# OmerMersin/video-stab

Measured on AMD Instinct MI355X. Metric: stabilized frames/sec @1080p (whole job; warp-stage HBM GB/s in roofline), higher is better.
Workload: dtype u8

## Files before the change

### video-stab_amd/csrc/batch_schedule.cpp

```cpp
#include <cstring>
#include <new>

#include "stab_internal.h"

using namespace vsd;

struct vs_batch {
    int device = 0, S = 0, B = 0, cap = 0;
    bool own = false;
    std::vector<vs_stab*> m;
    vs_stab* ref = nullptr;
    std::string err;
    FirstFailure failure;
    hipStream_t st = nullptr, st_pre = nullptr, st_det = nullptr, st_up = nullptr;
    bool allocated = false;
    uint8_t* h_tables = nullptr;
    size_t h_set_bytes = 0, ho_pairs = 0, ho_lk = 0, ho_rs = 0, ho_tail = 0, ho_gf = 0, ho_seg = 0;
    uint8_t* d_all = nullptr;
    uint8_t *d_lk[2] = {nullptr, nullptr}, *d_rs[2] = {nullptr, nullptr}, *d_tail[2] = {nullptr, nullptr}, *d_seg[2] = {nullptr, nullptr}, *d_gf = nullptr;
    uint8_t* d_tin[2] = {nullptr, nullptr};
    ImgPair* d_pairs[2] = {nullptr, nullptr};
    size_t up_bytes = 0;
    int pre_rel_step = -1;
    double* d_MinvB[2] = {nullptr, nullptr};
// ... 190 lines not shown
};

int fill_stream_items(vs_batch* g, vs_stab* s, const vs_batch::HostSet& H, const BorderPlan& bp, int ndue, int first, StepPlan& P) {
    const vs_params_c& p = s->p;
    const int ns = (int)s->bq.size(), dset = g->dev_set(P.k), set = g->pend_set;
    vs_batch::Ready& R = g->next;
    int npad = 0;
    for (int i = 0; i < ns; i++) {
        const int idx = first + i;
        const vs_stab::BFrame& b = s->bq[i];
        const vs_stab::ItemBufs& it = s->items[i];
        LKLevel L[MAX_PYR];
        fill_lk_levels(s, b.pv, b.c, L);
        const int cap = std::max(b.lk_cap, 0);
        P.n_max = std::max(P.n_max, cap);
        uint8_t *rs = H.rs + ransac_item_bytes() * idx, *tail = H.tail + tail_item_bytes() * idx;
        VS_OBJ_TRY(g, lk_fill_item(H.lk + lk_item_bytes() * idx, L, s->levels, s->d_pts[b.lk_buf], cap, s->d_npts[b.lk_buf], it.next, it.status, it.err,
                              p.lk_win_size, p.lk_max_iters, p.lk_epsilon));
        VS_OBJ_TRY(g, ransac_fill_item(rs, s->d_pts[b.lk_buf], it.next, it.status, cap, s->d_npts[b.lk_buf], it.vp, it.vc, it.m, 4, p.ransac_threshold,
                                  p.ransac_max_iters, s->tab, it.counts, it.model, it.inliers, it.info, s->d_traj, &s->tp, s->d_dbg, b.have_prev_gray));
        ransac_item_set_last(rs, i == ns - 1 ? 1 : 0);
        ransac_item_set_tail_in(rs, g->d_tin[dset] + tail_in_bytes() * idx);
        double* minv = nullptr;
        WarpTabJob jobs[2] = {{nullptr, nullptr, nullptr, 0, 0}, {nullptr, nullptr, nullptr, 0, 0}};
        if (b.out_due) {
            const int j = P.npend++;
            minv = g->d_MinvB[set] + 12 * j;
            R.srcs[j] = b.out_frame; R.dsts[j] = b.d_out; R.slots[j] = b.out_slot; R.owner[j] = s; R.pad_idx[j] = npad;
            if (P.all_apart && std::min(WARP_BATCH_MAX, ndue - j / WARP_BATCH_MAX * WARP_BATCH_MAX) >= WARP_TAB_MIN) {
                const WarpEnds e = warp_ends(s, b.out_frame, b.d_out, npad, bp);
                int32_t* T = g->d_tabs[set] + (size_t)j * g->tab_ints;
                jobs[0] = WarpTabJob{T, e.src, e.dst, bp.pw, bp.ph};
                if (fmt_two_planes(s->fmt))
                    jobs[1] = WarpTabJob{T + tab_layout(s->w, s->h).stride, e.src + src_uv(s), e.dst + dst_uv(s, e.dst, b.out_stride), s->w / 2, s->h / 2};
                else if (fmt_three_planes(s->fmt))
                    jobs[1] = WarpTabJob{T + tab_layout(s->w, s->h).stride, e.src + src_i420(s).u, e.dst + dst_i420(s, e.dst, b.out_stride).u, s->w / 2, s->h / 2};
            }
            npad++;
            P.pend_stride = b.out_stride;
        }
        tail_fill_item(tail, b.out_due ? 1 : 0, b.out_idx, minv, jobs);
        tail_item_set_seg(tail, P.nseg);
    }
    tail_fill_seg(H.seg + tail_seg_bytes() * P.nseg, first, ns, s->d_M, s->d_traj, s->d_dbg, p.smoothing_method);
    P.any_apart |= p.smoothing_method != VS_SMOOTH_KALMAN;
    P.nseg++;
    return VS_OK;
}

void fill_pair_tables(const vs_batch* g, const std::vector<vs_stab*>& act, ImgPair* h_pairs, StepPlan& P) {
    const int L = g->ref->levels;
    int n_first = 0, n_rest = 0, i = 0;
    for (vs_stab* s : act)
        for (const vs_stab::BFrame& b : s->bq) {
            const Pyramid& py = s->pyr[b.c];
            const int slot = b.detect ? n_first++ : P.ndet + n_rest++;
            h_pairs[slot] = ImgPair{b.frame, py.img[0]};
            if ((uintptr_t)b.frame % 8) P.aligned = 0;
            for (int l = 1; l <= L; l++) h_pairs[(size_t)l * P.n + i] = ImgPair{py.img[l - 1], py.img[l]};
// ... 356 lines not shown
```

### video-stab_amd/csrc/k_ransac.hip

```cpp
#include <map>
#include <mutex>
#include <vector>

#include <cstring>

#include "traj_device.h"
#include "traj_emit_device.h"
#include "vs_common.h"
#include "warp_tab.h"

namespace vsd {

struct RansacTables {
    int max_m = 0, iters = 0;
    uint32_t* d_pairs = nullptr;
    uint32_t* d_update = nullptr;
};

namespace {

struct CvRng {
    uint64_t state;
    explicit CvRng(uint64_t s) : state(s ? s : 0xffffffffULL) {}
    uint32_t next() {
// ... 508 lines not shown
                     iters, tab, d_counts, d_model, d_inliers, d_info, traj, tp, dbg, have_prev_gray);
    return VS_OK;
}

int launch_ransac_score_batch(const void* d_table, int items, int iters, int n_max, hipStream_t st) {
    if (!d_table || items < 1 || items > 65535 || iters < 1 || n_max < 0 || n_max > MAX_PTS) {
        set_last_error("ransac_score_batch: invalid argument");
        return VS_ERR_INVALID_ARG;
    }
    hipLaunchKernelGGL(ransac_score16_batch_kernel, dim3((iters + SC_HYP - 1) / SC_HYP, items), dim3(64), (size_t)(n_max > 0 ? n_max : 1) * 16, st,
                       static_cast<const RansacArgs*>(d_table));
    hipLaunchKernelGGL(ransac_select_batch_kernel, dim3(items), dim3(64), 0, st, static_cast<const RansacArgs*>(d_table), items - 1);
    VS_HIP_TRY(hipGetLastError());
    return VS_OK;
}

size_t tail_item_bytes() { return sizeof(TailItem); }

void tail_fill_item(void* host_item, int out_due, int out_idx, double* d_Minv_out, const WarpTabJob* tabs) {
    TailItem& t = *static_cast<TailItem*>(host_item);
    t.out_due = out_due; t.out_idx = out_idx; t.Minv_out = d_Minv_out; t.ncnt = 0; t.seg = 0;
    for (int i = 0; i < 2; i++) {
        if (tabs) t.tab[i] = tabs[i];
        else { t.tab[i].tabs = nullptr; t.tab[i].src = nullptr; t.tab[i].dst = nullptr; t.tab[i].dw = 0; t.tab[i].dh = 0; }
    }
}

size_t tail_seg_bytes() { return sizeof(TailSeg); }
void tail_fill_seg(void* host_seg, int first, int n, float* d_M_out, TrajState* traj, vs_debug_frame* dbg, int smoothing_method) {
    TailSeg& g = *static_cast<TailSeg*>(host_seg);
    g.first = first; g.n = n; g.M_out = d_M_out; g.traj = traj; g.dbg = dbg;
    g.apart = smoothing_method != VS_SMOOTH_KALMAN ? 1 : 0; g.pad = 0;
}
size_t tail_in_bytes() { return sizeof(TailIn); }
void tail_in_fill(void* host_tail_in, const double* model, int ok, int nprev, int have_prev_gray) {
    TailIn& t = *static_cast<TailIn*>(host_tail_in);
    memset(&t, 0, sizeof t);
    for (int i = 0; i < 6; i++) t.model[i] = ok ? model[i] : __builtin_nan("");
    t.info[0] = ok; t.info[1] = ok ? 0 : -1;
    t.nprev = nprev; t.have_prev_gray = have_prev_gray;
}
void ransac_fill_item_traj(void* host_item, TrajState* traj, const TrajParams* tp, vs_debug_frame* dbg) {
    RansacArgs& a = *static_cast<RansacArgs*>(host_item);
    memset(&a, 0, sizeof a);
    a.traj = traj; a.tp = *tp; a.dbg = dbg; a.have_prev_gray = 1;
}
void ransac_item_set_tail_in(void* host_item, void* d_tail_in) { static_cast<RansacArgs*>(host_item)->tail_in = static_cast<TailIn*>(d_tail_in); }
// ... 58 lines not shown
```

### video-stab_amd/csrc/k_warp.hip

```cpp
#include <algorithm>
#include <cstdlib>
#include <map>
#include <mutex>
#include <utility>
#include <vector>

#include "launchers.h"
#include "vs_common.h"
#include "warp_tab.h"

namespace vsd {

namespace {

constexpr int TW = WT_TW;
constexpr int TH = WT_TH;
constexpr int PX = 4;
constexpr int NT = 256;
constexpr int TXN = TW / PX;
constexpr int TYN = NT / TXN;
constexpr int MAXB = WARP_BATCH_MAX;
constexpr int FDATA = 136;
constexpr int FPITCH = 136;
constexpr int FROWS = 25;
constexpr int LDS_PX = FPITCH * FROWS;
constexpr int SG = FDATA / 4;
constexpr int SR = 7;
constexpr int SPASS = (FROWS + SR - 1) / SR;
constexpr int LUT_STRIDE = 32;
constexpr int OBUF = (NT / 64) * 2 * TW;

struct WarpCore {
    size_t sstride, dstride;
    int sw, sh, dw, dh;
    int src_aligned, dst_aligned;
    int border;
};

struct WarpArgs {
    WarpCore c;
    const double* Minv_dev;
    double Minv_val[MAXB * 6];
    int minv_stride;
    int32_t* tabs;
    int tab_stride;
    int tab_row, tab_ad;
    const uint8_t* srcs[MAXB];
    uint8_t* dsts[MAXB];
};

template <int CN, int SB = 1>
__device__ __forceinline__ uint32_t load_px_checked(const uint8_t* src, size_t sstride, int sw,
                                                    int sh, int sx, int sy, int border = VS_BORDER_BLACK) {
    if (border == VS_BORDER_REPLICATE) {
        sx = sx < 0 ? 0 : (sx >= sw ? sw - 1 : sx);
        sy = sy < 0 ? 0 : (sy >= sh ? sh - 1 : sy);
    } else if ((unsigned)sx >= (unsigned)sw || (unsigned)sy >= (unsigned)sh) return 0u;
    if (SB == 2) {
        const uint16_t* q = reinterpret_cast<const uint16_t*>(src + (size_t)sy * sstride) + (size_t)sx * CN;
        uint32_t v16 = q[0];
        if (CN > 1) v16 |= (uint32_t)q[1] << 16;
        return v16;
    }
    const uint8_t* p = src + (size_t)sy * sstride + (size_t)sx * CN;
    uint32_t v = p[0];
    if (CN > 1) v |= (uint32_t)p[1] << 8;
    if (CN > 2) v |= (uint32_t)p[2] << 16;
    if (CN > 3) v |= (uint32_t)p[3] << 24;
    return v;
// ... 272 lines not shown
}

__device__ __forceinline__ int coord_term(double p, double q, double v) { return wt_coord_term(p, q, v); }

__device__ __forceinline__ void load_map(const WarpArgs& a, int bz, double* m) {
    if (a.Minv_dev) {
        const __attribute__((address_space(4))) double* mp =
            (const __attribute__((address_space(4))) double*)(a.Minv_dev + a.minv_stride * bz);
#pragma unroll
        for (int i = 0; i < 6; i++) m[i] = mp[i];
    } else {
#pragma unroll
        for (int i = 0; i < 6; i++) m[i] = a.Minv_val[6 * bz + i];
    }
}

constexpr int TAB_COL = WT_COL;

__global__ __launch_bounds__(NT) void warp_tables_kernel(WarpArgs a) {
    const int bz = blockIdx.y;
    double m[6];
    load_map(a, bz, m);
    TabLayout L;
    L.row = a.tab_row; L.ad = a.tab_ad; L.stride = a.tab_stride;
    const int j = blockIdx.x * NT + threadIdx.x;
    if (j < wt_entries(a.c.dw, a.c.dh))
        wt_build_entry(a.tabs + (size_t)bz * a.tab_stride, L, m, a.c.dw, a.c.dh, a.srcs[bz], a.dsts[bz], j);
}

constexpr int NVT_MAX = 16;
struct NvTabArgs {
    int32_t* tabs;
    int block, chroma;
    int w, h;
    size_t src_uv, dst_uv;
    const uint8_t* ys[NVT_MAX];
    uint8_t* yd[NVT_MAX];
    double my[NVT_MAX * 6], muv[NVT_MAX * 6];
};

__global__ __launch_bounds__(NT) void warp_tables_nv12_kernel(NvTabArgs a) {
    const int bz = blockIdx.y, plane = blockIdx.z;
    const int dw = plane ? a.w / 2 : a.w, dh = plane ? a.h / 2 : a.h;
    TabLayout L = tab_layout(dw, dh);
    L.stride = a.block;
    double m[6];
#pragma unroll
    for (int i = 0; i < 6; i++) m[i] = plane ? a.muv[6 * bz + i] : a.my[6 * bz + i];
    const int j = blockIdx.x * NT + threadIdx.x;
    if (j < wt_entries(dw, dh))
// ... 36 lines not shown
        } else if (tid < 2 * 64 + TH) {
            const int r = min(y0 + (tid - 128), y1);
            tv0 = Tg[2 * a.c.dw + r]; tv1 = Tg[2 * a.c.dw + a.c.dh + r];
        }
    } else {
        double m[6];
        load_map(a, bz, m);
        if (wave < 2) {
            const double dv = (double)min(x0 + tid, x1);
            s_ad[tid] = coord_term(m[0], 0.0, dv);
            s_bd[tid] = coord_term(m[3], 0.0, dv);
        } else if (tid < 2 * 64 + TH) {
            const double dv = (double)min(y0 + (tid - 128), y1);
            s_x0[tid - 128] = coord_term(m[1], m[2], dv) + 16;
            s_y0[tid - 128] = coord_term(m[4], m[5], dv) + 16;
        }
        __syncthreads();
        const int cl = x1 - x0, rl = y1 - y0;
        ad0 = __builtin_amdgcn_readfirstlane(s_ad[0]); ad1 = __builtin_amdgcn_readfirstlane(s_ad[cl]);
        bd0 = __builtin_amdgcn_readfirstlane(s_bd[0]); bd1 = __builtin_amdgcn_readfirstlane(s_bd[cl]);
        Xa = __builtin_amdgcn_readfirstlane(s_x0[0]); Xb = __builtin_amdgcn_readfirstlane(s_x0[rl]);
        Ya = __builtin_amdgcn_readfirstlane(s_y0[0]); Yb = __builtin_amdgcn_readfirstlane(s_y0[rl]);
    }
    int bx0, bx1, by0, by1;
    bool saturated;
    {
        const int sx00 = (Xa + ad0) >> 10, sx01 = (Xa + ad1) >> 10, sx10 = (Xb + ad0) >> 10, sx11 = (Xb + ad1) >> 10;
        const int sy00 = (Ya + bd0) >> 10, sy01 = (Ya + bd1) >> 10, sy10 = (Yb + bd0) >> 10, sy11 = (Yb + bd1) >> 10;
        const int rx0 = min(min(sx00, sx01), min(sx10, sx11)), rx1 = max(max(sx00, sx01), max(sx10, sx11));
        const int ry0 = min(min(sy00, sy01), min(sy10, sy11)), ry1 = max(max(sy00, sy01), max(sy10, sy11));
        saturated = rx0 < -32768 || ry0 < -32768 || rx1 > 32767 || ry1 > 32767;
        bx0 = max(rx0, -32768); bx1 = min(rx1, 32767) + 1;
        by0 = max(ry0, -32768); by1 = min(ry1, 32767) + 1;
    }
    const int bx0a = bx0 & ~3;
    const int bw = (bx1 - bx0a + 1 + 3) & ~3;
    const int bh = by1 - by0 + 1;
    const bool fast = CN == 3 && !saturated && bw <= FDATA && bh <= FROWS;
    const bool use_lds = fast || (!saturated && (long long)bw * bh <= LDS_PX);
    const bool interior = fast && a.c.src_aligned && bx0a >= 0 && bx0a + bw <= a.c.sw && by0 >= 0 && by0 + bh <= a.c.sh &&
                          (bx0a + bw + 2 <= a.c.sw || by0 + bh < a.c.sh);

    if (interior) {
        const int ly = tid / SG, lx = tid - ly * SG;
        if (tid < SG * SR && 4 * lx < bw) {
            const uint8_t* box = src + (size_t)bx0a * 3 + (size_t)by0 * a.c.sstride;
            const uint32_t stride32 = (uint32_t)a.c.sstride, col = 12u * lx;
            U4 d[SPASS];
#pragma unroll
            for (int k = 0; k < SPASS; k++)
                if (SR * k < bh)
                    d[k] = *reinterpret_cast<const U4*>(box + (__umul24((uint32_t)min(ly + SR * k, bh - 1), stride32) + col));
#pragma unroll
            for (int k = 0; k < SPASS; k++) {
                if (SR * k < bh && (SR * (k + 1) <= FROWS || ly + SR * k < FROWS))
                    *reinterpret_cast<uint4*>(&tile[(ly + SR * k) * FPITCH + 4 * lx]) =
                        make_uint4(__builtin_amdgcn_perm(d[k].a, d[k].a, 0x02010300u),
                                   __builtin_amdgcn_perm(d[k].b, d[k].a, 0x05040603u),
                                   __builtin_amdgcn_perm(d[k].c, d[k].b, 0x04030502u),
                                   __builtin_amdgcn_perm(d[k].d, d[k].c, 0x03020401u));
            }
        }
    } else if (use_lds) {
        const int pitch = fast ? FPITCH : bw;
// ... 59 lines not shown
        const double dv = (double)min(y0 + (tid - TW), y1);
        s_x0[tid - TW] = coord_term(j.m[1], j.m[2], dv) + 16;
        s_y0[tid - TW] = coord_term(j.m[4], j.m[5], dv) + 16;
    }
    __syncthreads();
    WarpCore c;
    c.sstride = j.sstride; c.dstride = j.dstride;
    c.sw = j.sw; c.sh = j.sh; c.dw = j.dw; c.dh = j.dh;
    c.src_aligned = 0;
    const int galign = j.cn == 2 ? 8 : 4;
    c.dst_aligned = ((uintptr_t)j.dst % galign == 0) && (j.dstride % galign == 0);
    c.border = j.border;
    if (j.cn == 1) emit_rows<1, false>(c, j.src, j.dst, nullptr, s_ad, s_bd, s_x0, s_y0, x0, y0, x1, y1, 0, 0, 0, tid);
    else if (j.cn == 2) emit_rows<2, false>(c, j.src, j.dst, nullptr, s_ad, s_bd, s_x0, s_y0, x0, y0, x1, y1, 0, 0, 0, tid);
    else emit_rows<3, false>(c, j.src, j.dst, nullptr, s_ad, s_bd, s_x0, s_y0, x0, y0, x1, y1, 0, 0, 0, tid);
}

constexpr int TABN = 2 * TW + 2 * TH;

typedef const __attribute__((address_space(1))) int32_t* gtab_t;
struct TabK {
    WarpCore c;
    gtab_t tabs;
    int tab_stride, tab_row, tab_ad;
    int gx, gy;
};

struct TileIn {
    const uint8_t* src;
    uint8_t* dst;
    int bz, x0, y0, x1, y1;
    int ad0, ad1, bd0, bd1, Xa, Xb, Ya, Yb;
};

struct TileBox { int bx0a, by0, bw, bh; bool fast, use_lds, interior, pre, slowcols; };

__device__ __forceinline__ TileBox tile_box(const WarpCore& c, const TileIn& t) {
    TileBox b;
    const int sx00 = (t.Xa + t.ad0) >> 10, sx01 = (t.Xa + t.ad1) >> 10, sx10 = (t.Xb + t.ad0) >> 10, sx11 = (t.Xb + t.ad1) >> 10;
    const int sy00 = (t.Ya + t.bd0) >> 10, sy01 = (t.Ya + t.bd1) >> 10, sy10 = (t.Yb + t.bd0) >> 10, sy11 = (t.Yb + t.bd1) >> 10;
    const int rx0 = min(min(sx00, sx01), min(sx10, sx11)), rx1 = max(max(sx00, sx01), max(sx10, sx11));
    const int ry0 = min(min(sy00, sy01), min(sy10, sy11)), ry1 = max(max(sy00, sy01), max(sy10, sy11));
    const bool saturated = rx0 < -32768 || ry0 < -32768 || rx1 > 32767 || ry1 > 32767;
    const int bx0 = max(rx0, -32768), bx1 = min(rx1, 32767) + 1;
    b.by0 = max(ry0, -32768);
    const int by1 = min(ry1, 32767) + 1;
    b.bx0a = bx0 & ~3;
    b.bw = (bx1 - b.bx0a + 1 + 3) & ~3;
    b.bh = by1 - b.by0 + 1;
    b.fast = !saturated && b.bw <= FDATA && b.bh <= FROWS;
    b.use_lds = b.fast || (!saturated && (long long)b.bw * b.bh <= LDS_PX);
    b.interior = b.fast && c.src_aligned && b.bx0a >= 0 && b.bx0a + b.bw <= c.sw && b.by0 >= 0 && b.by0 + b.bh <= c.sh &&
                 (b.bx0a + b.bw + 2 <= c.sw || b.by0 + b.bh < c.sh);
    b.pre = b.fast && c.src_aligned && c.sw >= 8;
    b.slowcols = !b.interior && (b.bx0a < 0 || b.bx0a + b.bw + 2 > c.sw) && ((c.sw & 3) != 0 || c.border == VS_BORDER_REPLICATE);
    return b;
}

struct TilePre { U4 d[SPASS]; int tv0, tv1; };

__device__ __forceinline__ void load_terms(const TabK& k, const TileIn& t, int tid, int& tv0, int& tv1) {
    gtab_t Tg = k.tabs + (size_t)t.bz * k.tab_stride + k.tab_ad;
    if (tid < TW) {
        const int c = min(t.x0 + tid, t.x1);
        tv0 = Tg[c]; tv1 = Tg[k.c.dw + c];
    } else if (tid < TW + TH) {
        const int r = min(t.y0 + (tid - TW), t.y1);
        tv0 = Tg[2 * k.c.dw + r]; tv1 = Tg[2 * k.c.dw + k.c.dh + r];
    }
}

__device__ __forceinline__ void store_terms(int* tab, int tid, int tv0, int tv1, int subx = 0, int suby = 0) {
    if (tid < TW) { tab[tid] = tv0; tab[TW + tid] = tv1; }
    else if (tid < TW + TH) { tab[2 * TW + (tid - TW)] = tv0 - subx; tab[2 * TW + TH + (tid - TW)] = tv1 - suby; }
}

__device__ __forceinline__ int edge_class(const WarpCore& c, int cg, bool row_ok) {
    if (!row_ok) return 2;
// ... 61 lines not shown
                }
                *reinterpret_cast<uint4*>(&tile[(ly + SR * q) * FPITCH + 4 * lx]) = e;
            }
        }
    }
    store_terms(tab, tid, pf.tv0, pf.tv1, b.bx0a << 10, b.by0 << 10);
}

struct TileId { int x, y, z; };
__device__ __forceinline__ TileId tile_id(uint32_t flags, uint32_t gx, uint32_t gy, uint32_t mgx, uint32_t mgy) {
    TileId t;
    if (!(flags & 0x100u)) { t.x = blockIdx.x; t.y = blockIdx.y; t.z = blockIdx.z; return t; }
    const uint32_t n = gx * gy * (flags >> 16);
    const uint32_t lin = blockIdx.x + gx * (blockIdx.y + gy * blockIdx.z);
    const uint32_t c = lin & 7u, k = lin >> 3, q = n >> 3, r = n & 7u;
    const uint32_t seq = c * q + (c < r ? c : r) + k;
    const uint32_t row = gx == 1 ? seq : __umulhi(seq, mgx);
    t.x = (int)(seq - row * gx);
    t.z = (int)(gy == 1 ? row : __umulhi(row, mgy));
    t.y = (int)(row - (uint32_t)t.z * gy);
    return t;
}

__global__ __launch_bounds__(NT, 8) void warp_tab_kernel(gtab_t tabs, int tab_stride, int tab_row, int tab_ad, uint32_t sstride, uint32_t dstride,
                                                      uint32_t swh, uint32_t dwh, uint32_t flags, uint32_t mgx, uint32_t mgy) {
    __shared__ __attribute__((aligned(16))) uint32_t tile[LDS_PX];
    __shared__ __attribute__((aligned(16))) uint32_t obuf[OBUF];
    __shared__ int s_tab[TABN];
    __shared__ __attribute__((aligned(16))) uint8_t lut[32 * LUT_STRIDE];
    typedef const __attribute__((address_space(4))) int32_t* cptr;
    typedef __attribute__((address_space(1))) uint8_t* gptr;
    const int tid = threadIdx.x;
    TabK k;
    k.c.sstride = sstride; k.c.dstride = dstride;
    k.c.sw = swh & 0xFFFFu; k.c.sh = swh >> 16; k.c.dw = dwh & 0xFFFFu; k.c.dh = dwh >> 16;
    k.c.src_aligned = flags & 1u; k.c.dst_aligned = (flags >> 1) & 1u; k.c.border = (flags >> 2) & 7u;
    k.tabs = tabs; k.tab_stride = tab_stride; k.tab_row = tab_row; k.tab_ad = tab_ad;
    k.gx = (k.c.dw + TW - 1) / TW; k.gy = (k.c.dh + TH - 1) / TH;
    TileIn cur;
    const TileId tq = tile_id(flags, (uint32_t)(k.c.dw + TW - 1) / TW, (uint32_t)(k.c.dh + TH - 1) / TH, mgx, mgy);
    {
        cptr Ts = (cptr)(const int32_t*)(tabs + (size_t)tq.z * tab_stride);
        typedef int32_t i32x8 __attribute__((ext_vector_type(8)));
        typedef int32_t i32x4 __attribute__((ext_vector_type(4)));
        const i32x8 cc = *(const __attribute__((address_space(4))) i32x8*)(Ts + TAB_COL * tq.x);
        const i32x4 cr = *(const __attribute__((address_space(4))) i32x4*)(Ts + tab_row + 4 * tq.y);
        cur.src = (const uint8_t*)(gptr)((unsigned long long)(uint32_t)cc[0] | (unsigned long long)(uint32_t)cc[1] << 32);
        cur.dst = (uint8_t*)(gptr)((unsigned long long)(uint32_t)cc[2] | (unsigned long long)(uint32_t)cc[3] << 32);
        cur.ad0 = cc[4]; cur.ad1 = cc[5]; cur.bd0 = cc[6]; cur.bd1 = cc[7];
        cur.Xa = cr[0]; cur.Xb = cr[1]; cur.Ya = cr[2]; cur.Yb = cr[3];
        cur.bz = tq.z; cur.x0 = tq.x * TW; cur.y0 = tq.y * TH;
        cur.x1 = min(cur.x0 + TW, k.c.dw) - 1; cur.y1 = min(cur.y0 + TH, k.c.dh) - 1;
    }
    if (tid >= NT - 32) {
        const uint32_t f = tid - (NT - 32);
        const uint32_t wlo = (32u - f) | (f << 8);
        *reinterpret_cast<uint4*>(lut + f * LUT_STRIDE) =
            make_uint4(wlo, wlo << 16, __float_as_uint((float)(32u - f) * 0x1p121f), __float_as_uint((float)f * 0x1p121f));
    }
    TilePre pf;
    pf.tv0 = 0; pf.tv1 = 0;
    load_terms(k, cur, tid, pf.tv0, pf.tv1);
    const TileBox cb = tile_box(k.c, cur);
    if (cb.pre) {
        issue_tile(k, cur, cb, tid, pf);
        store_tile(k, cur, cb, tid, pf, tile, s_tab);
    } else {
        const int tv0 = pf.tv0, tv1 = pf.tv1;
        if (cb.use_lds) {
            const int pitch = cb.fast ? FPITCH : cb.bw;
            const int gpr = cb.bw >> 2;
            const int total = gpr * cb.bh;
            for (int g = tid; g < total; g += NT) {
                const int row = g / gpr, gxx = g - row * gpr;
                uint4 px = stage_group<3>(k.c, cur.src, cb.bx0a + 4 * gxx, cb.by0 + row);
                if (cb.fast) {
                    const uint32_t nx = load_px_checked<3>(cur.src, k.c.sstride, k.c.sw, k.c.sh, cb.bx0a + 4 * gxx + 4, cb.by0 + row, k.c.border);
                    px = make_uint4(pair_b(px.x, px.y), pair_b(px.y, px.z), pair_b(px.z, px.w), pair_b(px.w, nx));
                }
                *reinterpret_cast<uint4*>(&tile[row * pitch + 4 * gxx]) = px;
            }
        }
        store_terms(s_tab, tid, tv0, tv1, cb.fast ? cb.bx0a << 10 : 0, cb.fast ? cb.by0 << 10 : 0);
    }
    __syncthreads();
    if (cb.fast) emit_fast(k.c, cur.dst, tile, obuf, lut, s_tab, s_tab + TW, s_tab + 2 * TW, s_tab + 2 * TW + TH, cur.x0, cur.y0, cur.x1, cur.y1, 0, tid);
// ... 412 lines not shown
    WarpCore c;
    c.border = (flags >> 2) & 7u;
    uint32_t gx, mgx;
    int sadd = 0, dadd = 0;
    if (t < n1) {
        c.sstride = sstride; c.dstride = dstride;
        c.sw = c.dw = w; c.sh = c.dh = h;
        c.src_aligned = flags & 1u; c.dst_aligned = (flags >> 1) & 1u;
        gx = gx1; mgx = mgx1;
    } else {
        t -= n1;
        if (t >= n2) { t -= n2; sadd = svu; dadd = dvu; }
        T += tab_layout(w, h).stride;
        c.sstride = scpitch; c.dstride = dcpitch;
        c.sw = c.dw = (int)w2; c.sh = c.dh = (int)h2;
        c.src_aligned = (flags >> 5) & 1u; c.dst_aligned = (flags >> 6) & 1u;
        gx = gx2; mgx = mgx2;
    }
    const TabLayout L = tab_layout(c.dw, c.dh);
    const uint32_t row = gx == 1 ? t : __umulhi(t, mgx);
    plane_tile<1, BORDER, SB>(c, (cptr)(const int32_t*)T, T + L.ad, L.row, (int)(t - row * gx), (int)row, tile, lut, s_row, threadIdx.x, sadd, dadd);
}

inline int tab_stride_of(int dw, int dh) { return tab_layout(dw, dh).stride; }

template <int CN>
void launch_one(WarpArgs& a, dim3 grid, int32_t* d_tabs, int what, hipStream_t st, int tab_stride, int sb) {
    a.tabs = d_tabs;
    const TabLayout tl = tab_layout(a.c.dw, a.c.dh);
    a.tab_stride = tab_stride > 0 ? tab_stride : tl.stride; a.tab_row = tl.row; a.tab_ad = tl.ad;
    if (sb == 2) {
        if (d_tabs && what != VS_WARP_ONLY)
            hipLaunchKernelGGL(warp_tables_kernel, dim3((a.c.dw + a.c.dh + grid.x + grid.y + NT - 1) / NT, grid.z), dim3(NT), 0, st, a);
        if (d_tabs && what == VS_WARP_TABLES_ONLY) return;
        if constexpr (CN <= 2) hipLaunchKernelGGL((warp_affine16_kernel<CN>), grid, dim3(NT), 0, st, a);
        return;
    }
    if (d_tabs) {
        if (what != VS_WARP_ONLY)
            hipLaunchKernelGGL(warp_tables_kernel, dim3((a.c.dw + a.c.dh + grid.x + grid.y + NT - 1) / NT, grid.z), dim3(NT), 0, st, a);
        if (what == VS_WARP_TABLES_ONLY) return;
        const bool packs = a.c.sw < 65536 && a.c.sh < 65536 && a.c.dw < 65536 && a.c.dh < 65536 && a.c.sstride < (1ull << 24) && a.c.dstride < (1ull << 24);
        auto order = [](const dim3& g, uint32_t* mgx, uint32_t* mgy) -> uint32_t {
            *mgx = (uint32_t)((0x100000000ull + g.x - 1) / g.x); *mgy = (uint32_t)((0x100000000ull + g.y - 1) / g.y);
            const unsigned long long n = (unsigned long long)g.x * g.y * g.z;
            return (g.x > 1 || g.y > 1) && n * std::max(g.x, g.y) < (1ull << 31) && g.z < 65536 ? (0x100u | (uint32_t)g.z << 16) : 0u;
        };
        uint32_t mgx = 0, mgy = 0;
        if (CN == 3 && packs) {
            const uint32_t of = order(grid, &mgx, &mgy);
            hipLaunchKernelGGL(warp_tab_kernel, grid, dim3(NT), 0, st, (gtab_t)a.tabs, a.tab_stride, a.tab_row, a.tab_ad, (uint32_t)a.c.sstride,
                               (uint32_t)a.c.dstride, (uint32_t)a.c.sw | (uint32_t)a.c.sh << 16, (uint32_t)a.c.dw | (uint32_t)a.c.dh << 16,
                               (uint32_t)(a.c.src_aligned ? 1 : 0) | (uint32_t)(a.c.dst_aligned ? 2 : 0) | (uint32_t)a.c.border << 2 | of, mgx, mgy);
        } else if (CN != 3 && packs && a.c.border == VS_BORDER_BLACK) {
            const dim3 pg(grid.x, (a.c.dh + PlaneCfg<CN>::THP - 1) / PlaneCfg<CN>::THP, grid.z);
            const uint32_t of = order(pg, &mgx, &mgy);
            hipLaunchKernelGGL((warp_plane_kernel<(CN == 3 ? 1 : CN)>), pg, dim3(NT), 0, st, (gtab_t)a.tabs, a.tab_stride, a.tab_row, a.tab_ad, (uint32_t)a.c.sstride,
                               (uint32_t)a.c.dstride, (uint32_t)a.c.sw | (uint32_t)a.c.sh << 16, (uint32_t)a.c.dw | (uint32_t)a.c.dh << 16,
                               (uint32_t)(a.c.src_aligned ? 1 : 0) | (uint32_t)(a.c.dst_aligned ? 2 : 0) | (uint32_t)a.c.border << 2 | of, mgx, mgy);
        } else {
            hipLaunchKernelGGL((warp_affine_kernel<CN, true>), grid, dim3(NT), 0, st, a);
        }
    } else {
        hipLaunchKernelGGL((warp_affine_kernel<CN, false>), grid, dim3(NT), 0, st, a);
    }
}

void launch_cn(WarpArgs& a, dim3 grid, int cn, int32_t* d_tabs, hipStream_t st, int what = VS_WARP_ALL, int tab_stride = 0, int sb = 1) {
    if (cn == 3) launch_one<3>(a, grid, d_tabs, what, st, tab_stride, sb);
    else if (cn == 4) launch_one<4>(a, grid, d_tabs, what, st, tab_stride, sb);
    else if (cn == 1) launch_one<1>(a, grid, d_tabs, what, st, tab_stride, sb);
    else launch_one<2>(a, grid, d_tabs, what, st, tab_stride, sb);
}

// ... 314 lines not shown
```

### video-stab_amd/csrc/warp_tab.h

```cpp
#ifndef VS_WARP_TAB_H
#define VS_WARP_TAB_H

#include <stdint.h>

namespace vsd {

constexpr int WT_TW = 128;
constexpr int WT_TH = 16;
constexpr int WT_COL = 8;

struct TabLayout { int row, ad, stride; };

#ifdef __HIPCC__
__host__ __device__
#endif
inline TabLayout tab_layout(int dw, int dh) {
    const int gx = (dw + WT_TW - 1) / WT_TW, gy = (dh + WT_TH - 1) / WT_TH;
    TabLayout t;
    t.row = WT_COL * gx;
    t.ad = t.row + 4 * gy;
    t.stride = (t.ad + 2 * dw + 2 * dh + 3) & ~3;
    return t;
}

inline int nv12_tab_ints(int w, int h) { return tab_layout(w, h).stride + tab_layout(w / 2, h / 2).stride; }

struct WarpTabJob {
    int32_t* tabs;
    const uint8_t* src;
    uint8_t* dst;
    int32_t dw, dh;
};

#ifdef __HIPCC__
__device__ __forceinline__ int wt_coord_term(double p, double q, double v) { return __double2int_rn((p * v + q) * 1024); }

__device__ __forceinline__ int wt_entries(int dw, int dh) { return dw + dh + (dw + WT_TW - 1) / WT_TW + (dh + WT_TH - 1) / WT_TH; }

__device__ __forceinline__ void wt_build_entry(int32_t* __restrict__ T, const TabLayout& L, const double* m, int dw, int dh,
                                               const uint8_t* src, uint8_t* dst, int j) {
    const int gx = (dw + WT_TW - 1) / WT_TW, gy = (dh + WT_TH - 1) / WT_TH;
    if (j < dw) {
        const double dv = (double)j;
        T[L.ad + j] = wt_coord_term(m[0], 0.0, dv);
        T[L.ad + dw + j] = wt_coord_term(m[3], 0.0, dv);
        return;
    }
    j -= dw;
    if (j < dh) {
        const double dv = (double)j;
        T[L.ad + 2 * dw + j] = wt_coord_term(m[1], m[2], dv) + 16;
        T[L.ad + 2 * dw + dh + j] = wt_coord_term(m[4], m[5], dv) + 16;
        return;
    }
    j -= dh;
    if (j < gx) {
        const int x1 = j * WT_TW + WT_TW < dw ? j * WT_TW + WT_TW : dw;
        const double v0 = (double)(j * WT_TW), v1 = (double)(x1 - 1);
        int32_t* C = T + WT_COL * j;
        *reinterpret_cast<const uint8_t**>(C) = src;
        *reinterpret_cast<uint8_t**>(C + 2) = dst;
        C[4] = wt_coord_term(m[0], 0.0, v0); C[5] = wt_coord_term(m[0], 0.0, v1);
        C[6] = wt_coord_term(m[3], 0.0, v0); C[7] = wt_coord_term(m[3], 0.0, v1);
        return;
    }
    j -= gx;
    if (j < gy) {
        const int y1 = j * WT_TH + WT_TH < dh ? j * WT_TH + WT_TH : dh;
        const double v0 = (double)(j * WT_TH), v1 = (double)(y1 - 1);
        int32_t* R = T + L.row + 4 * j;
        R[0] = wt_coord_term(m[1], m[2], v0) + 16; R[1] = wt_coord_term(m[1], m[2], v1) + 16;
        R[2] = wt_coord_term(m[4], m[5], v0) + 16; R[3] = wt_coord_term(m[4], m[5], v1) + 16;
    }
}

__device__ __forceinline__ void wt_build_plane(const WarpTabJob& job, const double* m, int tid, int nthreads) {
    if (!job.tabs) return;
    const TabLayout L = tab_layout(job.dw, job.dh);
    const int n = wt_entries(job.dw, job.dh);
    for (int j = tid; j < n; j += nthreads) wt_build_entry(job.tabs, L, m, job.dw, job.dh, job.src, job.dst, j);
}
#endif

}
#endif
```

Measured before the change: 127,200.

## Precompute per-tile source boxes in warp tables for BGR warp kernel

Adds a per-tile box section to the warp tables that holds the source bounding box and fast/LDS/inside/xover flags, computed once when the tables are built. The BGR table-driven warp kernel then reads one packed 16-byte record per tile instead of loading column/row endpoint terms and recomputing the box. This moves the box arithmetic out of the hot warp kernel and shrinks its table loads, in exchange for larger tables and a bit more work in the table builder. The shared box logic is factored into a header helper used by both paths.

```diff
diff --git a/video-stab_amd/csrc/batch_schedule.cpp b/video-stab_amd/csrc/batch_schedule.cpp
--- a/video-stab_amd/csrc/batch_schedule.cpp
+++ b/video-stab_amd/csrc/batch_schedule.cpp
@@ -236,7 +236,7 @@
         ransac_item_set_last(rs, i == ns - 1 ? 1 : 0);
         ransac_item_set_tail_in(rs, g->d_tin[dset] + tail_in_bytes() * idx);
         double* minv = nullptr;
-        WarpTabJob jobs[2] = {{nullptr, nullptr, nullptr, 0, 0}, {nullptr, nullptr, nullptr, 0, 0}};
+        WarpTabJob jobs[2] = {{nullptr, nullptr, nullptr, 0, 0, 0, 0, 0}, {nullptr, nullptr, nullptr, 0, 0, 0, 0, 0}};
         if (b.out_due) {
             const int j = P.npend++;
             minv = g->d_MinvB[set] + 12 * j;
@@ -244,11 +244,11 @@
             if (P.all_apart && std::min(WARP_BATCH_MAX, ndue - j / WARP_BATCH_MAX * WARP_BATCH_MAX) >= WARP_TAB_MIN) {
                 const WarpEnds e = warp_ends(s, b.out_frame, b.d_out, npad, bp);
                 int32_t* T = g->d_tabs[set] + (size_t)j * g->tab_ints;
-                jobs[0] = WarpTabJob{T, e.src, e.dst, bp.pw, bp.ph};
+                jobs[0] = WarpTabJob{T, e.src, e.dst, bp.pw, bp.ph, s->cn == 3 && fmt_sample_bytes(s->fmt) == 1 && !fmt_two_planes(s->fmt) && !fmt_three_planes(s->fmt) ? WT_TH : 0, bp.pw, bp.ph};
                 if (fmt_two_planes(s->fmt))
-                    jobs[1] = WarpTabJob{T + tab_layout(s->w, s->h).stride, e.src + src_uv(s), e.dst + dst_uv(s, e.dst, b.out_stride), s->w / 2, s->h / 2};
+                    jobs[1] = WarpTabJob{T + tab_layout(s->w, s->h).stride, e.src + src_uv(s), e.dst + dst_uv(s, e.dst, b.out_stride), s->w / 2, s->h / 2, 0, s->w / 2, s->h / 2};
                 else if (fmt_three_planes(s->fmt))
-                    jobs[1] = WarpTabJob{T + tab_layout(s->w, s->h).stride, e.src + src_i420(s).u, e.dst + dst_i420(s, e.dst, b.out_stride).u, s->w / 2, s->h / 2};
+                    jobs[1] = WarpTabJob{T + tab_layout(s->w, s->h).stride, e.src + src_i420(s).u, e.dst + dst_i420(s, e.dst, b.out_stride).u, s->w / 2, s->h / 2, 0, s->w / 2, s->h / 2};
             }
             npad++;
             P.pend_stride = b.out_stride;
diff --git a/video-stab_amd/csrc/k_ransac.hip b/video-stab_amd/csrc/k_ransac.hip
--- a/video-stab_amd/csrc/k_ransac.hip
+++ b/video-stab_amd/csrc/k_ransac.hip
@@ -554,7 +554,7 @@
     t.out_due = out_due; t.out_idx = out_idx; t.Minv_out = d_Minv_out; t.ncnt = 0; t.seg = 0;
     for (int i = 0; i < 2; i++) {
         if (tabs) t.tab[i] = tabs[i];
-        else { t.tab[i].tabs = nullptr; t.tab[i].src = nullptr; t.tab[i].dst = nullptr; t.tab[i].dw = 0; t.tab[i].dh = 0; }
+        else { t.tab[i].tabs = nullptr; t.tab[i].src = nullptr; t.tab[i].dst = nullptr; t.tab[i].dw = 0; t.tab[i].dh = 0; t.tab[i].th = 0; t.tab[i].sw = 0; t.tab[i].sh = 0; }
     }
 }
 
diff --git a/video-stab_amd/csrc/k_warp.hip b/video-stab_amd/csrc/k_warp.hip
--- a/video-stab_amd/csrc/k_warp.hip
+++ b/video-stab_amd/csrc/k_warp.hip
@@ -45,6 +45,7 @@
     int32_t* tabs;
     int tab_stride;
     int tab_row, tab_ad;
+    int tab_box, tab_th;
     const uint8_t* srcs[MAXB];
     uint8_t* dsts[MAXB];
 };
@@ -363,10 +364,10 @@
     double m[6];
     load_map(a, bz, m);
     TabLayout L;
-    L.row = a.tab_row; L.ad = a.tab_ad; L.stride = a.tab_stride;
+    L.row = a.tab_row; L.ad = a.tab_ad; L.box = a.tab_box; L.stride = a.tab_stride;
     const int j = blockIdx.x * NT + threadIdx.x;
-    if (j < wt_entries(a.c.dw, a.c.dh))
-        wt_build_entry(a.tabs + (size_t)bz * a.tab_stride, L, m, a.c.dw, a.c.dh, a.srcs[bz], a.dsts[bz], j);
+    if (j < wt_entries(a.c.dw, a.c.dh, a.tab_th))
+        wt_build_entry(a.tabs + (size_t)bz * a.tab_stride, L, m, a.c.dw, a.c.dh, a.srcs[bz], a.dsts[bz], j, a.tab_th, a.c.sw, a.c.sh);
 }
 
 constexpr int NVT_MAX = 16;
@@ -449,24 +450,11 @@
         Xa = __builtin_amdgcn_readfirstlane(s_x0[0]); Xb = __builtin_amdgcn_readfirstlane(s_x0[rl]);
         Ya = __builtin_amdgcn_readfirstlane(s_y0[0]); Yb = __builtin_amdgcn_readfirstlane(s_y0[rl]);
     }
-    int bx0, bx1, by0, by1;
-    bool saturated;
-    {
-        const int sx00 = (Xa + ad0) >> 10, sx01 = (Xa + ad1) >> 10, sx10 = (Xb + ad0) >> 10, sx11 = (Xb + ad1) >> 10;
-        const int sy00 = (Ya + bd0) >> 10, sy01 = (Ya + bd1) >> 10, sy10 = (Yb + bd0) >> 10, sy11 = (Yb + bd1) >> 10;
-        const int rx0 = min(min(sx00, sx01), min(sx10, sx11)), rx1 = max(max(sx00, sx01), max(sx10, sx11));
-        const int ry0 = min(min(sy00, sy01), min(sy10, sy11)), ry1 = max(max(sy00, sy01), max(sy10, sy11));
-        saturated = rx0 < -32768 || ry0 < -32768 || rx1 > 32767 || ry1 > 32767;
-        bx0 = max(rx0, -32768); bx1 = min(rx1, 32767) + 1;
-        by0 = max(ry0, -32768); by1 = min(ry1, 32767) + 1;
-    }
-    const int bx0a = bx0 & ~3;
-    const int bw = (bx1 - bx0a + 1 + 3) & ~3;
-    const int bh = by1 - by0 + 1;
-    const bool fast = CN == 3 && !saturated && bw <= FDATA && bh <= FROWS;
-    const bool use_lds = fast || (!saturated && (long long)bw * bh <= LDS_PX);
-    const bool interior = fast && a.c.src_aligned && bx0a >= 0 && bx0a + bw <= a.c.sw && by0 >= 0 && by0 + bh <= a.c.sh &&
-                          (bx0a + bw + 2 <= a.c.sw || by0 + bh < a.c.sh);
+    const WtBox wb = wt_tile_box(ad0, ad1, bd0, bd1, Xa, Xb, Ya, Yb, a.c.sw, a.c.sh, WT_STAGE_BGR);
+    const int bx0a = wb.bx0a, by0 = wb.by0, bw = wb.bw, bh = wb.bh;
+    const bool fast = CN == 3 && (wb.flags & WT_BOX_FAST);
+    const bool use_lds = (wb.flags & WT_BOX_LDS) != 0;
+    const bool interior = fast && a.c.src_aligned && (wb.flags & WT_BOX_INSIDE);
 
     if (interior) {
         const int ly = tid / SG, lx = tid - ly * SG;
@@ -572,7 +560,7 @@
 struct TabK {
     WarpCore c;
     gtab_t tabs;
-    int tab_stride, tab_row, tab_ad;
+    int tab_stride, tab_box, tab_ad;
     int gx, gy;
 };
 
@@ -580,30 +568,18 @@
     const uint8_t* src;
     uint8_t* dst;
     int bz, x0, y0, x1, y1;
-    int ad0, ad1, bd0, bd1, Xa, Xb, Ya, Yb;
 };
 
 struct TileBox { int bx0a, by0, bw, bh; bool fast, use_lds, interior, pre, slowcols; };
 
-__device__ __forceinline__ TileBox tile_box(const WarpCore& c, const TileIn& t) {
+__device__ __forceinline__ TileBox tile_box(const WarpCore& c, const WtBox& w) {
     TileBox b;
-    const int sx00 = (t.Xa + t.ad0) >> 10, sx01 = (t.Xa + t.ad1) >> 10, sx10 = (t.Xb + t.ad0) >> 10, sx11 = (t.Xb + t.ad1) >> 10;
-    const int sy00 = (t.Ya + t.bd0) >> 10, sy01 = (t.Ya + t.bd1) >> 10, sy10 = (t.Yb + t.bd0) >> 10, sy11 = (t.Yb + t.bd1) >> 10;
-    const int rx0 = min(min(sx00, sx01), min(sx10, sx11)), rx1 = max(max(sx00, sx01), max(sx10, sx11));
-    const int ry0 = min(min(sy00, sy01), min(sy10, sy11)), ry1 = max(max(sy00, sy01), max(sy10, sy11));
-    const bool saturated = rx0 < -32768 || ry0 < -32768 || rx1 > 32767 || ry1 > 32767;
-    const int bx0 = max(rx0, -32768), bx1 = min(rx1, 32767) + 1;
-    b.by0 = max(ry0, -32768);
-    const int by1 = min(ry1, 32767) + 1;
-    b.bx0a = bx0 & ~3;
-    b.bw = (bx1 - b.bx0a + 1 + 3) & ~3;
-    b.bh = by1 - b.by0 + 1;
-    b.fast = !saturated && b.bw <= FDATA && b.bh <= FROWS;
-    b.use_lds = b.fast || (!saturated && (long long)b.bw * b.bh <= LDS_PX);
-    b.interior = b.fast && c.src_aligned && b.bx0a >= 0 && b.bx0a + b.bw <= c.sw && b.by0 >= 0 && b.by0 + b.bh <= c.sh &&
-                 (b.bx0a + b.bw + 2 <= c.sw || b.by0 + b.bh < c.sh);
+    b.bx0a = w.bx0a; b.by0 = w.by0; b.bw = w.bw; b.bh = w.bh;
+    b.fast = (w.flags & WT_BOX_FAST) != 0;
+    b.use_lds = (w.flags & WT_BOX_LDS) != 0;
+    b.interior = (w.flags & WT_BOX_INSIDE) && c.src_aligned;
     b.pre = b.fast && c.src_aligned && c.sw >= 8;
-    b.slowcols = !b.interior && (b.bx0a < 0 || b.bx0a + b.bw + 2 > c.sw) && ((c.sw & 3) != 0 || c.border == VS_BORDER_REPLICATE);
+    b.slowcols = !b.interior && (w.flags & WT_BOX_XOVER) && ((c.sw & 3) != 0 || c.border == VS_BORDER_REPLICATE);
     return b;
 }
 
@@ -711,7 +687,7 @@
     return t;
 }
 
-__global__ __launch_bounds__(NT, 8) void warp_tab_kernel(gtab_t tabs, int tab_stride, int tab_row, int tab_ad, uint32_t sstride, uint32_t dstride,
+__global__ __launch_bounds__(NT, 8) void warp_tab_kernel(gtab_t tabs, int tab_stride, int tab_box, int tab_ad, uint32_t sstride, uint32_t dstride,
                                                       uint32_t swh, uint32_t dwh, uint32_t flags, uint32_t mgx, uint32_t mgy) {
     __shared__ __attribute__((aligned(16))) uint32_t tile[LDS_PX];
     __shared__ __attribute__((aligned(16))) uint32_t obuf[OBUF];
@@ -724,20 +700,19 @@
     k.c.sstride = sstride; k.c.dstride = dstride;
     k.c.sw = swh & 0xFFFFu; k.c.sh = swh >> 16; k.c.dw = dwh & 0xFFFFu; k.c.dh = dwh >> 16;
     k.c.src_aligned = flags & 1u; k.c.dst_aligned = (flags >> 1) & 1u; k.c.border = (flags >> 2) & 7u;
-    k.tabs = tabs; k.tab_stride = tab_stride; k.tab_row = tab_row; k.tab_ad = tab_ad;
+    k.tabs = tabs; k.tab_stride = tab_stride; k.tab_box = tab_box; k.tab_ad = tab_ad;
     k.gx = (k.c.dw + TW - 1) / TW; k.gy = (k.c.dh + TH - 1) / TH;
     TileIn cur;
+    WtBox rec;
     const TileId tq = tile_id(flags, (uint32_t)(k.c.dw + TW - 1) / TW, (uint32_t)(k.c.dh + TH - 1) / TH, mgx, mgy);
     {
         cptr Ts = (cptr)(const int32_t*)(tabs + (size_t)tq.z * tab_stride);
-        typedef int32_t i32x8 __attribute__((ext_vector_type(8)));
         typedef int32_t i32x4 __attribute__((ext_vector_type(4)));
-        const i32x8 cc = *(const __attribute__((address_space(4))) i32x8*)(Ts + TAB_COL * tq.x);
-        const i32x4 cr = *(const __attribute__((address_space(4))) i32x4*)(Ts + tab_row + 4 * tq.y);
+        const i32x4 cc = *(const __attribute__((address_space(4))) i32x4*)(Ts + TAB_COL * tq.x);
+        const i32x4 cr = *(const __attribute__((address_space(4))) i32x4*)(Ts + tab_box + 4 * (tq.y * k.gx + tq.x));
         cur.src = (const uint8_t*)(gptr)((unsigned long long)(uint32_t)cc[0] | (unsigned long long)(uint32_t)cc[1] << 32);
         cur.dst = (uint8_t*)(gptr)((unsigned long long)(uint32_t)cc[2] | (unsigned long long)(uint32_t)cc[3] << 32);
-        cur.ad0 = cc[4]; cur.ad1 = cc[5]; cur.bd0 = cc[6]; cur.bd1 = cc[7];
-        cur.Xa = cr[0]; cur.Xb = cr[1]; cur.Ya = cr[2]; cur.Yb = cr[3];
+        rec = wt_box_unpack(cr[0], cr[1], cr[2], cr[3]);
         cur.bz = tq.z; cur.x0 = tq.x * TW; cur.y0 = tq.y * TH;
         cur.x1 = min(cur.x0 + TW, k.c.dw) - 1; cur.y1 = min(cur.y0 + TH, k.c.dh) - 1;
     }
@@ -750,7 +725,7 @@
     TilePre pf;
     pf.tv0 = 0; pf.tv1 = 0;
     load_terms(k, cur, tid, pf.tv0, pf.tv1);
-    const TileBox cb = tile_box(k.c, cur);
+    const TileBox cb = tile_box(k.c, rec);
     if (cb.pre) {
         issue_tile(k, cur, cb, tid, pf);
         store_tile(k, cur, cb, tid, pf, tile, s_tab);
@@ -1209,23 +1184,25 @@
     plane_tile<1, BORDER, SB>(c, (cptr)(const int32_t*)T, T + L.ad, L.row, (int)(t - row * gx), (int)row, tile, lut, s_row, threadIdx.x, sadd, dadd);
 }
 
-inline int tab_stride_of(int dw, int dh) { return tab_layout(dw, dh).stride; }
+inline int tab_stride_of(int dw, int dh) { return tab_layout(dw, dh, TH).stride; }
 
 template <int CN>
 void launch_one(WarpArgs& a, dim3 grid, int32_t* d_tabs, int what, hipStream_t st, int tab_stride, int sb) {
     a.tabs = d_tabs;
-    const TabLayout tl = tab_layout(a.c.dw, a.c.dh);
-    a.tab_stride = tab_stride > 0 ? tab_stride : tl.stride; a.tab_row = tl.row; a.tab_ad = tl.ad;
+    a.tab_th = CN == 3 && sb == 1 ? TH : 0;
+    const TabLayout tl = tab_layout(a.c.dw, a.c.dh, a.tab_th);
+    const int tab_blocks = (a.c.dw + a.c.dh + (int)grid.x + (int)grid.y + (a.tab_th ? (int)(grid.x * grid.y) : 0) + NT - 1) / NT;
+    a.tab_stride = tab_stride > 0 ? tab_stride : tab_stride_of(a.c.dw, a.c.dh); a.tab_row = tl.row; a.tab_ad = tl.ad; a.tab_box = tl.box;
     if (sb == 2) {
         if (d_tabs && what != VS_WARP_ONLY)
-            hipLaunchKernelGGL(warp_tables_kernel, dim3((a.c.dw + a.c.dh + grid.x + grid.y + NT - 1) / NT, grid.z), dim3(NT), 0, st, a);
+            hipLaunchKernelGGL(warp_tables_kernel, dim3(tab_blocks, grid.z), dim3(NT), 0, st, a);
         if (d_tabs && what == VS_WARP_TABLES_ONLY) return;
         if constexpr (CN <= 2) hipLaunchKernelGGL((warp_affine16_kernel<CN>), grid, dim3(NT), 0, st, a);
         return;
     }
     if (d_tabs) {
         if (what != VS_WARP_ONLY)
-            hipLaunchKernelGGL(warp_tables_kernel, dim3((a.c.dw + a.c.dh + grid.x + grid.y + NT - 1) / NT, grid.z), dim3(NT), 0, st, a);
+            hipLaunchKernelGGL(warp_tables_kernel, dim3(tab_blocks, grid.z), dim3(NT), 0, st, a);
         if (what == VS_WARP_TABLES_ONLY) return;
         const bool packs = a.c.sw < 65536 && a.c.sh < 65536 && a.c.dw < 65536 && a.c.dh < 65536 && a.c.sstride < (1ull << 24) && a.c.dstride < (1ull << 24);
         auto order = [](const dim3& g, uint32_t* mgx, uint32_t* mgy) -> uint32_t {
@@ -1236,7 +1213,7 @@
         uint32_t mgx = 0, mgy = 0;
         if (CN == 3 && packs) {
             const uint32_t of = order(grid, &mgx, &mgy);
-            hipLaunchKernelGGL(warp_tab_kernel, grid, dim3(NT), 0, st, (gtab_t)a.tabs, a.tab_stride, a.tab_row, a.tab_ad, (uint32_t)a.c.sstride,
+            hipLaunchKernelGGL(warp_tab_kernel, grid, dim3(NT), 0, st, (gtab_t)a.tabs, a.tab_stride, a.tab_box, a.tab_ad, (uint32_t)a.c.sstride,
                                (uint32_t)a.c.dstride, (uint32_t)a.c.sw | (uint32_t)a.c.sh << 16, (uint32_t)a.c.dw | (uint32_t)a.c.dh << 16,
                                (uint32_t)(a.c.src_aligned ? 1 : 0) | (uint32_t)(a.c.dst_aligned ? 2 : 0) | (uint32_t)a.c.border << 2 | of, mgx, mgy);
         } else if (CN != 3 && packs && a.c.border == VS_BORDER_BLACK) {
diff --git a/video-stab_amd/csrc/warp_tab.h b/video-stab_amd/csrc/warp_tab.h
--- a/video-stab_amd/csrc/warp_tab.h
+++ b/video-stab_amd/csrc/warp_tab.h
@@ -9,18 +9,76 @@
 constexpr int WT_TH = 16;
 constexpr int WT_COL = 8;
 
-struct TabLayout { int row, ad, stride; };
+struct TabLayout { int row, ad, box, stride; };
 
 #ifdef __HIPCC__
 __host__ __device__
 #endif
-inline TabLayout tab_layout(int dw, int dh) {
+inline TabLayout tab_layout(int dw, int dh, int th = 0) {
     const int gx = (dw + WT_TW - 1) / WT_TW, gy = (dh + WT_TH - 1) / WT_TH;
     TabLayout t;
     t.row = WT_COL * gx;
     t.ad = t.row + 4 * gy;
-    t.stride = (t.ad + 2 * dw + 2 * dh + 3) & ~3;
+    t.box = (t.ad + 2 * dw + 2 * dh + 3) & ~3;
+    t.stride = t.box + (th > 0 ? 4 * gx * ((dh + th - 1) / th) : 0);
     return t;
+}
+
+struct WtStage { int max_w, max_rows, lds_px; };
+constexpr WtStage WT_STAGE_BGR = {136, 25, 136 * 25};
+
+enum : uint32_t {
+    WT_BOX_FAST = 1u,
+    WT_BOX_LDS = 2u,
+    WT_BOX_INSIDE = 4u,
+    WT_BOX_XOVER = 8u,
+    WT_BOX_SAT = 16u,
+};
+
+struct WtBox { int bx0a, by0, bw, bh; uint32_t flags; };
+
+#ifdef __HIPCC__
+__host__ __device__
+#endif
+inline WtBox wt_tile_box(int ad0, int ad1, int bd0, int bd1, int Xa, int Xb, int Ya, int Yb, int sw, int sh, const WtStage& st) {
+    const int sx00 = (Xa + ad0) >> 10, sx01 = (Xa + ad1) >> 10, sx10 = (Xb + ad0) >> 10, sx11 = (Xb + ad1) >> 10;
+    const int sy00 = (Ya + bd0) >> 10, sy01 = (Ya + bd1) >> 10, sy10 = (Yb + bd0) >> 10, sy11 = (Yb + bd1) >> 10;
+    const int ax0 = sx00 < sx01 ? sx00 : sx01, ax1 = sx10 < sx11 ? sx10 : sx11, cx0 = sx00 > sx01 ? sx00 : sx01, cx1 = sx10 > sx11 ? sx10 : sx11;
+    const int ay0 = sy00 < sy01 ? sy00 : sy01, ay1 = sy10 < sy11 ? sy10 : sy11, cy0 = sy00 > sy01 ? sy00 : sy01, cy1 = sy10 > sy11 ? sy10 : sy11;
+    const int rx0 = ax0 < ax1 ? ax0 : ax1, rx1 = cx0 > cx1 ? cx0 : cx1, ry0 = ay0 < ay1 ? ay0 : ay1, ry1 = cy0 > cy1 ? cy0 : cy1;
+    const bool saturated = rx0 < -32768 || ry0 < -32768 || rx1 > 32767 || ry1 > 32767;
+    const int bx0 = rx0 > -32768 ? rx0 : -32768, bx1 = (rx1 < 32767 ? rx1 : 32767) + 1;
+    const int by1 = (ry1 < 32767 ? ry1 : 32767) + 1;
+    WtBox b;
+    b.by0 = ry0 > -32768 ? ry0 : -32768;
+    b.bx0a = bx0 & ~3;
+    b.bw = (bx1 - b.bx0a + 1 + 3) & ~3;
+    b.bh = by1 - b.by0 + 1;
+    const bool fast = !saturated && b.bw <= st.max_w && b.bh <= st.max_rows;
+    const bool lds = fast || (!saturated && (long long)b.bw * b.bh <= st.lds_px);
+    const bool inside = fast && b.bx0a >= 0 && b.bx0a + b.bw <= sw && b.by0 >= 0 && b.by0 + b.bh <= sh &&
+                        (b.bx0a + b.bw + 2 <= sw || b.by0 + b.bh < sh);
+    const bool xover = b.bx0a < 0 || b.bx0a + b.bw + 2 > sw;
+    b.flags = (fast ? WT_BOX_FAST : 0u) | (lds ? WT_BOX_LDS : 0u) | (inside ? WT_BOX_INSIDE : 0u) | (xover ? WT_BOX_XOVER : 0u) |
+              (saturated ? WT_BOX_SAT : 0u);
+    return b;
+}
+
+#ifdef __HIPCC__
+__host__ __device__
+#endif
+inline void wt_box_pack(const WtBox& b, int32_t* r) {
+    const uint32_t bw = b.bw < 65535 ? (uint32_t)b.bw : 65535u, bh = b.bh < 65535 ? (uint32_t)b.bh : 65535u;
+    r[0] = b.bx0a; r[1] = b.by0; r[2] = (int32_t)(bw | bh << 16); r[3] = (int32_t)b.flags;
+}
+
+#ifdef __HIPCC__
+__host__ __device__
+#endif
+inline WtBox wt_box_unpack(int r0, int r1, int r2, int r3) {
+    WtBox b;
+    b.bx0a = r0; b.by0 = r1; b.bw = (int)((uint32_t)r2 & 0xFFFFu); b.bh = (int)((uint32_t)r2 >> 16); b.flags = (uint32_t)r3;
+    return b;
 }
 
 inline int nv12_tab_ints(int w, int h) { return tab_layout(w, h).stride + tab_layout(w / 2, h / 2).stride; }
@@ -30,15 +88,19 @@
     const uint8_t* src;
     uint8_t* dst;
     int32_t dw, dh;
+    int32_t th, sw, sh;
 };
 
 #ifdef __HIPCC__
 __device__ __forceinline__ int wt_coord_term(double p, double q, double v) { return __double2int_rn((p * v + q) * 1024); }
 
-__device__ __forceinline__ int wt_entries(int dw, int dh) { return dw + dh + (dw + WT_TW - 1) / WT_TW + (dh + WT_TH - 1) / WT_TH; }
+__device__ __forceinline__ int wt_entries(int dw, int dh, int th = 0) {
+    const int gx = (dw + WT_TW - 1) / WT_TW;
+    return dw + dh + gx + (dh + WT_TH - 1) / WT_TH + (th > 0 ? gx * ((dh + th - 1) / th) : 0);
+}
 
 __device__ __forceinline__ void wt_build_entry(int32_t* __restrict__ T, const TabLayout& L, const double* m, int dw, int dh,
-                                               const uint8_t* src, uint8_t* dst, int j) {
+                                               const uint8_t* src, uint8_t* dst, int j, int th = 0, int sw = 0, int sh = 0) {
     const int gx = (dw + WT_TW - 1) / WT_TW, gy = (dh + WT_TH - 1) / WT_TH;
     if (j < dw) {
         const double dv = (double)j;
@@ -71,14 +133,25 @@
         int32_t* R = T + L.row + 4 * j;
         R[0] = wt_coord_term(m[1], m[2], v0) + 16; R[1] = wt_coord_term(m[1], m[2], v1) + 16;
         R[2] = wt_coord_term(m[4], m[5], v0) + 16; R[3] = wt_coord_term(m[4], m[5], v1) + 16;
+        return;
+    }
+    j -= gy;
+    if (th > 0 && j < gx * ((dh + th - 1) / th)) {
+        const int ty = j / gx, tx = j - ty * gx;
+        const int x1 = tx * WT_TW + WT_TW < dw ? tx * WT_TW + WT_TW : dw, y1 = ty * th + th < dh ? ty * th + th : dh;
+        const double c0 = (double)(tx * WT_TW), c1 = (double)(x1 - 1), r0 = (double)(ty * th), r1 = (double)(y1 - 1);
+        const WtBox b = wt_tile_box(wt_coord_term(m[0], 0.0, c0), wt_coord_term(m[0], 0.0, c1), wt_coord_term(m[3], 0.0, c0), wt_coord_term(m[3], 0.0, c1),
+                                    wt_coord_term(m[1], m[2], r0) + 16, wt_coord_term(m[1], m[2], r1) + 16, wt_coord_term(m[4], m[5], r0) + 16,
+                                    wt_coord_term(m[4], m[5], r1) + 16, sw, sh, WT_STAGE_BGR);
+        wt_box_pack(b, T + L.box + 4 * j);
     }
 }
 
 __device__ __forceinline__ void wt_build_plane(const WarpTabJob& job, const double* m, int tid, int nthreads) {
     if (!job.tabs) return;
-    const TabLayout L = tab_layout(job.dw, job.dh);
-    const int n = wt_entries(job.dw, job.dh);
-    for (int j = tid; j < n; j += nthreads) wt_build_entry(job.tabs, L, m, job.dw, job.dh, job.src, job.dst, j);
+    const TabLayout L = tab_layout(job.dw, job.dh, job.th);
+    const int n = wt_entries(job.dw, job.dh, job.th);
+    for (int j = tid; j < n; j += nthreads) wt_build_entry(job.tabs, L, m, job.dw, job.dh, job.src, job.dst, j, job.th, job.sw, job.sh);
 }
 #endif
 
```

New measurement: 126,000, median of 2. No clear change (-0.9%).
